# JohannesErnst/WeaSAL

Measured on AMD Instinct MI355X. Metric: points/sec fwd+bwd KPFCNN on DALES spheres; achieved HBM GB/s on KPConv gather, higher is better.
Workload: dtype f32; 1 GPU; DALES_PseudoLabel KP-FCNN, in_radius=10m, 50k pts/sphere, batch=8, fp32, step = GPU pyramid + fwd + loss + bwd + SGD; contrast_loss term included (trainer_PseudoLabel.py:204-208); pyramid of the next batch overlapped on a second stream; parallelism=dp1, dist_world_size=1, allreduce_bytes=0

## Files before the change

### include/weasal_hip.h

```cpp
#ifndef WEASAL_HIP_H
#define WEASAL_HIP_H

#include <stdint.h>

#ifdef __cplusplus
extern "C" {
#endif

typedef enum {
    WS_OK = 0,
    WS_ERR_INVALID = 1,
    WS_ERR_UNSUPPORTED = 2,
    WS_ERR_HIP = 3,
    WS_ERR_EMPTY = 4,
    WS_ERR_CAPACITY = 5
} ws_status;

enum { WS_INFLUENCE_LINEAR = 0, WS_INFLUENCE_CONSTANT = 1, WS_INFLUENCE_GAUSSIAN = 2 };
enum { WS_AGGREGATION_SUM = 0, WS_AGGREGATION_CLOSEST = 1 };

const char* ws_last_error(void);
int64_t ws_launch_count(void);
const char* ws_version(void);
int ws_device_count(void);
// ... 382 lines not shown
                      int32_t lut_n, const float* class_w, const float* grad_loss, const float* wsum, float* dlogits, int64_t ldd,
                      void* stream);
int ws_sgd_step(float* const* h_params, const float* const* h_grads, float* const* h_bufs, const int64_t* h_sizes, int32_t count,
                float lr, float momentum, float weight_decay, float clip_value, int32_t first, void* stream);

int ws_kpconv_deform_prepare(const float* offset_features, int64_t n, int32_t od, const float* kernel_points, int32_t k,
                             float extent, int32_t modulated, float* deformed_kp, float* modulations, float* kp4, float* kp_rmax,
                             void* stream);
int ws_kpconv_deform_prepare_bwd(const float* d_kp4, const float* d_deformed_kp, const float* kp4, int64_t n, int32_t od, int32_t k,
                                 float extent, int32_t modulated, float* d_offset_features, void* stream);
int ws_kpconv_gather_fwd_def(const float* q_pts, int64_t nq, const float* s_pts, int64_t ns, const int64_t* inds, int32_t h,
                             const void* x, int32_t ci, const float* kp4, int32_t k, float extent, const int32_t* order,
                             void* wf, float* min_d2, int32_t rows_bf16, int32_t rows_sorted, void* stream);
int ws_kpconv_gather_fwd_ex(const float* q_pts, int64_t nq, const float* s_pts, int64_t ns, const int64_t* inds, int32_t h,
                            const void* x, int32_t ci, const float* kernel_points, int32_t k, const float* deformed_kp,
                            const float* modulations, float extent, int32_t influence, int32_t aggregation, const int32_t* order,
                            void* wf, float* min_d2, int32_t rows_bf16, int32_t rows_sorted, void* stream);
int ws_kpconv_gather_bwd_x_def(const float* q_pts, int64_t nq, const float* s_pts, int64_t ns, int32_t h,
                               const int32_t* t_offsets, const int32_t* t_pairs, const void* dwf, int32_t ci, const float* kp4,
                               int32_t k, float extent, const int32_t* order, void* dx, int32_t rows_bf16, void* stream);
int ws_kpconv_gather_bwd_x_grid_wide(const float* s_pts, int64_t ns, const void* grid_blob, int32_t nb, int64_t cells,
                                     const uint64_t* key_last, float radius, const void* dwf, int32_t ci,
                                     const float* kernel_points, int32_t k, const float* kp4, const float* kp_rmax, float extent,
                                     const int32_t* order, const int64_t* rows, int32_t rows_h, void* dx, int32_t rows_bf16,
                                     void* stream);
int ws_kpconv_gather_bwd_geom_def(const float* q_pts, int64_t nq, const float* s_pts, int64_t ns, const int64_t* inds, int32_t h,
                                  const void* x, int32_t ci, const void* dwf, const float* kp4, int32_t k, const float* d_min_d2,
                                  float extent, const int32_t* order, float* d_kp4, int32_t rows_bf16, int32_t rows_sorted,
                                  void* stream);
int ws_kpconv_layer_fwd_fused(const float* q_pts, int64_t nq, const float* s_pts, int64_t ns, const int64_t* inds, int32_t h,
                              const float* x, int32_t ci, const float* kernel_points, int32_t k, float extent,
                              const int32_t* order, const float* weights, int32_t co, const float* bias, int32_t act, float slope,
                              float* out, void* stream);
int ws_kpconv_gather_fwd_variant(int32_t ci, int32_t mode, int32_t influence, int32_t aggregation, int32_t rows_bf16,
                                 int32_t rows_sorted, char* out, int32_t cap);
enum {
    WS_GATHER_FWD = 0, WS_GATHER_BWD_X = 1, WS_GATHER_BWD_GEOM = 2, WS_GATHER_BWD_X_GRID = 3,
    WS_GATHER_FWD_DEF = 4, WS_GATHER_BWD_X_DEF = 5, WS_GATHER_BWD_X_GRID_WIDE = 6, WS_GATHER_BWD_GEOM_DEF = 7
};
int ws_kpconv_gather_variant(int32_t op, int64_t nq, int64_t ns, int32_t ci, const void* rows_a, const void* rows_b, int32_t deformed,
                             int32_t modulated, int32_t influence, int32_t aggregation, int32_t rows_bf16, int32_t rows_sorted,
                             int32_t ordered, char* out, int32_t cap);
int ws_gemm_xb_variant(const float* x, int64_t m, int32_t k, int64_t ldx, const float* b, int64_t b_row_stride, int64_t b_col_stride,
                       int32_t n, const float* bias, const float* residual, int64_t ldr, const float* gate_y, int64_t ldg,
                       const uint8_t* mask, int64_t ldm, const float* y, int64_t ldy, const void* scratch, int64_t scratch_bytes,
                       char* out, int32_t cap);
int ws_gemm_xty_variant(const void* x, int64_t m, int32_t k, int64_t ldx, const void* y, int32_t n, int64_t ldy, float* out_m,
                        int64_t ldo, void* scratch, int32_t rows_bf16, char* out, int32_t cap);
int ws_act_bwd_colsum_variant(const float* dy, int64_t m, int32_t n, int64_t lddy, const float* y, int64_t ldy, const float* dz,
                              int64_t lddz, float* colsum, void* scratch, char* out, int32_t cap);
int ws_gemm_xbt_bf16_variant(int64_t m, int32_t k, int32_t n, const float* bias, const uint16_t* residual, int64_t ldr, const void* y,
                             int64_t ldy, int32_t out_f32, char* out, int32_t cap);
int ws_act_bwd_colsum_bf16_variant(int32_t dy_f32, int64_t m, int32_t n, float* colsum, void* scratch, char* out, int32_t cap);
int64_t ws_p2p_regularizer_scratch_bytes(int64_t n);
int ws_p2p_regularizer_fwd(const float* deformed_kp, const float* kp4, const float* min_d2, int64_t n, int32_t k, float extent,
                           float repulse_extent, float* out2, void* scratch, void* stream);
int ws_p2p_regularizer_bwd(const float* deformed_kp, const float* kp4, const float* min_d2, int64_t n, int32_t k, float extent,
                           float repulse_extent, const float* g2, float* d_min_d2, float* d_deformed_kp, void* stream);

#ifdef __cplusplus
}
#endif
#endif
```

### weasal_amd/_lib.py

```python
import ctypes as C
import os

_HERE = os.path.dirname(os.path.abspath(__file__))
LIB_PATH = os.path.join(_HERE, "libweasal_hip.so")

_vp = C.c_void_p
_i32 = C.c_int32
_i64 = C.c_int64
_f32 = C.c_float

SIGNATURES = {
    "ws_last_error": (C.c_char_p, []),
    "ws_version": (C.c_char_p, []),
    "ws_device_count": (C.c_int, []),
    "ws_kpconv_gather_fwd": (C.c_int, [_vp, _i64, _vp, _i64, _vp, _i32, _vp, _i32, _vp, _i32, _vp, _vp,
                                      _f32, _i32, _i32, _vp, _vp, _vp, _vp]),
    "ws_kpconv_gather_bwd_x": (C.c_int, [_vp, _i64, _vp, _i64, _vp, _i32, _vp, _vp, _vp, _i32, _vp, _i32,
                                        _vp, _vp, _f32, _i32, _i32, _vp, _vp, _vp]),
    "ws_kpconv_gather_bwd_geom": (C.c_int, [_vp, _i64, _vp, _i64, _vp, _i32, _vp, _i32, _vp, _vp, _i32,
                                           _vp, _vp, _vp, _f32, _i32, _i32, _vp, _vp, _vp]),
    "ws_transpose_scratch_bytes": (_i64, [_i64, _i32, _i64]),
    "ws_transpose_build": (C.c_int, [_vp, _i64, _i32, _i64, _vp, _vp, _vp, _vp]),
    "ws_max_pool_fwd": (C.c_int, [_vp, _i64, _i32, _vp, _i64, _i32, _vp, _vp, _vp]),
    "ws_max_pool_bwd": (C.c_int, [_vp, _vp, _i64, _i32, _i32, _vp, _vp, _i64, _vp, _vp]),
# ... 103 lines not shown
    "ws_anchor_scratch_bytes": (_i64, [_i64]),
    "ws_anchor_members_plan": (C.c_int, [_vp, _vp, _i64, _i32, _vp, _i64, C.c_double, _vp, _vp, _vp, _vp, _vp, _vp, _vp, _vp, _vp,
                                        _vp, _vp]),
    "ws_anchor_members_fill": (C.c_int, [_vp, _i64, _vp, _i64, C.c_double, _vp, _vp, _vp, _vp, _vp, _vp, _vp, _i64, _i64, _vp, _vp,
                                        _vp, _vp, _vp, _vp, _vp]),
    "ws_anchor_pairs_plan": (C.c_int, [_vp, _i64, _vp, _i64, C.c_double, _vp, _vp, _vp, _vp, _vp, _vp, _vp, _vp, _vp]),
    "ws_anchor_pairs_fill": (C.c_int, [_vp, _i64, _vp, _i64, C.c_double, _vp, _vp, _vp, _vp, _i64, _vp, _vp, _vp]),
    "ws_anchor_overlap_plan": (C.c_int, [_vp, _vp, _i64, _vp, _i64, _vp, _i64, _vp, _vp, _i64, _vp, _vp, _vp, _vp, _vp, _vp, _vp]),
    "ws_anchor_overlap_fill": (C.c_int, [_vp, _i64, _vp, _vp, _i64, _vp, _vp, _i64, _vp, _i64, _vp, _vp, _i64, _vp, _vp, _vp, _vp,
                                        _i64, _i64, _i64, _vp, _vp, _vp, _vp, _vp]),
    "ws_sampler_create": (C.c_int, [C.POINTER(_vp)]),
    "ws_sampler_destroy": (None, [_vp]),
    "ws_sampler_add_cloud": (C.c_int, [_vp, _vp, _vp, _i64, _vp, _vp, _i64, _vp]),
    "ws_sampler_state_bytes": (_i64, []),
    "ws_sampler_draw_bytes": (_i64, []),
    "ws_sampler_batch": (C.c_int, [_vp, _vp, _i32, _i32, _i64, C.c_double, _f32, C.c_uint64, C.c_uint64, _i32, _vp, _i32, _i32, _i32,
                                   _vp, _vp, _vp, _vp, _vp, _vp, _vp, _vp, _vp, _i64, _vp, _vp]),
    "ws_softmax_ce_scratch_bytes": (_i64, [_i64]),
    "ws_softmax_ce_fwd": (C.c_int, [_vp, _i64, _i32, _i64, _vp, _vp, _i32, _vp, _vp, _vp, _vp, _vp]),
    "ws_softmax_ce_bwd": (C.c_int, [_vp, _i64, _i32, _i64, _vp, _vp, _i32, _vp, _vp, _vp, _vp, _i64, _vp]),
    "ws_sgd_step": (C.c_int, [_vp, _vp, _vp, _vp, _i32, _f32, _f32, _f32, _f32, _i32, _vp]),
    "ws_kpconv_deform_prepare": (C.c_int, [_vp, _i64, _i32, _vp, _i32, _f32, _i32, _vp, _vp, _vp, _vp, _vp]),
    "ws_kpconv_gather_fwd_ex": (C.c_int, [_vp, _i64, _vp, _i64, _vp, _i32, _vp, _i32, _vp, _i32, _vp, _vp, _f32, _i32, _i32, _vp,
                                         _vp, _vp, _i32, _i32, _vp]),
    "ws_kpconv_deform_prepare_bwd": (C.c_int, [_vp, _vp, _vp, _i64, _i32, _i32, _f32, _i32, _vp, _vp]),
    "ws_kpconv_gather_fwd_def": (C.c_int, [_vp, _i64, _vp, _i64, _vp, _i32, _vp, _i32, _vp, _i32, _f32, _vp, _vp, _vp, _i32, _i32, _vp]),
    "ws_kpconv_gather_bwd_x_def": (C.c_int, [_vp, _i64, _vp, _i64, _i32, _vp, _vp, _vp, _i32, _vp, _i32, _f32, _vp, _vp, _i32, _vp]),
    "ws_kpconv_gather_bwd_x_grid_wide": (C.c_int, [_vp, _i64, _vp, _i32, _i64, _vp, _f32, _vp, _i32, _vp, _i32, _vp, _vp, _f32, _vp,
                                                   _vp, _i32, _vp, _i32, _vp]),
    "ws_kpconv_gather_bwd_geom_def": (C.c_int, [_vp, _i64, _vp, _i64, _vp, _i32, _vp, _i32, _vp, _vp, _i32, _vp, _f32, _vp, _vp,
                                                _i32, _i32, _vp]),
    "ws_kpconv_layer_fwd_fused": (C.c_int, [_vp, _i64, _vp, _i64, _vp, _i32, _vp, _i32, _vp, _i32, _f32, _vp, _vp, _i32, _vp, _i32, _f32,
                                           _vp, _vp]),
    "ws_kpconv_gather_fwd_variant": (C.c_int, [_i32, _i32, _i32, _i32, _i32, _i32, C.c_char_p, _i32]),
    "ws_kpconv_gather_variant": (C.c_int, [_i32, _i64, _i64, _i32, _vp, _vp, _i32, _i32, _i32, _i32, _i32, _i32, _i32, C.c_char_p, _i32]),
    "ws_gemm_xb_variant": (C.c_int, [_vp, _i64, _i32, _i64, _vp, _i64, _i64, _i32, _vp, _vp, _i64, _vp, _i64, _vp, _i64, _vp, _i64,
                                     _vp, _i64, C.c_char_p, _i32]),
    "ws_gemm_xty_variant": (C.c_int, [_vp, _i64, _i32, _i64, _vp, _i32, _i64, _vp, _i64, _vp, _i32, C.c_char_p, _i32]),
    "ws_act_bwd_colsum_variant": (C.c_int, [_vp, _i64, _i32, _i64, _vp, _i64, _vp, _i64, _vp, _vp, C.c_char_p, _i32]),
    "ws_gemm_xbt_bf16_variant": (C.c_int, [_i64, _i32, _i32, _vp, _vp, _i64, _vp, _i64, _i32, C.c_char_p, _i32]),
    "ws_act_bwd_colsum_bf16_variant": (C.c_int, [_i32, _i64, _i32, _vp, _vp, C.c_char_p, _i32]),
    "ws_p2p_regularizer_scratch_bytes": (_i64, [_i64]),
    "ws_p2p_regularizer_fwd": (C.c_int, [_vp, _vp, _vp, _i64, _i32, _f32, _f32, _vp, _vp, _vp]),
    "ws_p2p_regularizer_bwd": (C.c_int, [_vp, _vp, _vp, _i64, _i32, _f32, _f32, _vp, _vp, _vp, _vp]),
    "ws_timer_reset": (C.c_int, []),
    "ws_timer_count": (C.c_int, []),
    "ws_timer_read": (C.c_int, [_i32, _vp, _vp, _vp, _vp]),
    "ws_timer_read_layer": (C.c_int, [_i32, _vp]),
}

ENV_SWITCHES = (
    ("WEASAL_NB_WIDE_CAPS", "ws_nb_wide_caps"),
    ("WEASAL_CLOSEST_BWD_VEC", "ws_closest_bwd_vec"),
    ("WEASAL_GEMM_STAGED", "ws_gemm_staged"),
    ("WEASAL_GEMM_SHALLOW", "ws_gemm_shallow"),
)

_lib = None


class WeasalHipError(RuntimeError):
    pass


def lib():
    global _lib
# ... 43 lines not shown
```

### weasal_amd/csrc/blocks.hip

```cpp
#include <vector>

#include "ws_common.h"

extern "C" int ws_block_gates = 1;
extern "C" int ws_block_gather_residual = 1;
extern "C" int64_t ws_block_side_rows = 0;
extern "C" int ws_block_fused_infer = 1;
extern "C" int ws_block_pool_order = 1;

namespace {

struct Side {
    hipStream_t st = nullptr;
    hipEvent_t fork[3] = {nullptr, nullptr, nullptr};
    hipEvent_t join = nullptr;
};
int side_for_current_device(Side** out)
{
    static Side sides[16];
    int dev = 0;
    WS_HIP(hipGetDevice(&dev));
    WS_REQUIRE(dev >= 0 && dev < 16, "device index %d out of range", dev);
    Side& sd = sides[dev];
    if (!sd.st) {
        hipStream_t st;
        WS_HIP(hipStreamCreateWithFlags(&st, hipStreamNonBlocking));
        for (auto& e : sd.fork) WS_HIP(hipEventCreateWithFlags(&e, hipEventDisableTiming));
        WS_HIP(hipEventCreateWithFlags(&sd.join, hipEventDisableTiming));
        sd.st = st;
    }
    *out = &sd;
    return WS_OK;
}

struct Arena {
    char* base;
    int64_t cap, off;
    Arena(void* b, int64_t c) : base((char*)b), cap(c), off(0) {}
    template <typename T> T* take(int64_t count)
    {
// ... 80 lines not shown
    if (d->w1) t = max3(t, ws_gemm_xb_scratch_bytes(d->ns, d->in_dim, d->conv_in), 0);
    if (d->w2) t = max3(t, ws_gemm_xb_scratch_bytes(d->nq, d->conv_out, d->out_dim), d->ws ? ws_gemm_xb_scratch_bytes(d->nq, d->in_dim, d->out_dim) : 0);
    return t;
}

int kpblock_fwd(const ws_kpblock* d, Arena& ar, hipStream_t st, bool run)
{
    const int64_t nq = d->nq, ns = d->ns;
    const Lin l1{d->w1, d->conv_in, d->in_dim, d->in_dim}, l2{d->w2, d->out_dim, d->conv_out, d->conv_out},
        lsc{d->ws, d->out_dim, d->in_dim, d->in_dim};
    float* tr1 = d->w1 ? ar.take<float>(l1.tr_floats()) : nullptr;
    float* tr2 = d->w2 ? ar.take<float>(l2.tr_floats()) : nullptr;
    float* trs = d->ws ? ar.take<float>(lsc.tr_floats()) : nullptr;
    float* sc = (d->w2 && d->ws) ? ar.take<float>(nq * d->out_dim) : nullptr;
    const int64_t tmp_bytes = kpblock_tmp_fwd(d);
    void* tmp = ar.take<char>(tmp_bytes > 16 ? tmp_bytes : 16);
    if (!run) return WS_OK;
    if (nq == 0) return WS_OK;
    const float* x1 = d->feat;
    if (d->w1) {
        WS_TRY(linear_fwd(l1, d->feat, ns, d->in_dim, d->b1, nullptr, 0, 1, d->slope, d->x1, tr1, tmp, tmp_bytes, st));
        x1 = d->x1;
    }
    TimerRec rec{};
    if (d->timed) {
        WS_HIP(hipEventCreate(&rec.a));
        WS_HIP(hipEventCreate(&rec.b));
        rec.nq = nq; rec.h = d->h; rec.ci = d->conv_in;
        WS_HIP(hipEventRecord(rec.a, st));
    }
    float* x2 = d->w2 ? d->x2 : d->out;
    const bool one_launch = d->infer && d->conv_in == 32 && d->conv_out == 32 && !d->rows_sorted && ((uintptr_t)x1 & 15u) == 0 &&
                            ((uintptr_t)d->wk & 15u) == 0 && ((uintptr_t)x2 & 15u) == 0 && ws_block_fused_infer;
    if (one_launch) {
        WS_TRY(ws_kpconv_layer_fwd_fused(d->q_pts, nq, d->s_pts, ns, d->inds, d->h, x1, d->conv_in, d->kernel_points, d->k, d->extent,
                                         d->order_q, d->wk, d->conv_out, d->bk, 1, d->slope, x2, st));
        if (d->timed) WS_HIP(hipEventRecord(rec.b, st));
    } else {
        WS_REQUIRE(d->wf, "wf buffer missing");
        WS_TRY(ws_kpconv_gather_fwd_ex(d->q_pts, nq, d->s_pts, ns, d->inds, d->h, x1, d->conv_in, d->kernel_points, d->k, nullptr,
                                       nullptr, d->extent, WS_INFLUENCE_LINEAR, WS_AGGREGATION_SUM, d->order_q, d->wf, nullptr, 0,
                                       d->rows_sorted, st));
        if (d->timed) WS_HIP(hipEventRecord(rec.b, st));
        WS_TRY(ws_gemm_xb_epilogue_strided(d->wf, nq, d->k * d->conv_in, (int64_t)d->k * d->conv_in, d->wk, d->conv_out, 1, d->conv_out,
                                           d->bk, nullptr, 0, 1, d->slope, x2, d->conv_out, tmp, tmp_bytes, st));
    }
    if (d->timed) {
        WS_HIP(hipEventCreate(&rec.c));
        WS_HIP(hipEventRecord(rec.c, st));
        timer_recs().push_back(rec);
    }
    if (!d->w2) return WS_OK;
    const float* sc_in = d->feat;
    if (d->strided) {
        if (arg_bytes(d))
            WS_TRY(ws_priv_max_pool_fwd_u8(d->feat, ns, d->in_dim, d->inds, nq, d->h, d->pooled, reinterpret_cast<uint8_t*>(d->arg),
                                           ws_block_pool_order ? d->order_q : nullptr, st));
        else
            WS_TRY(ws_max_pool_fwd(d->feat, ns, d->in_dim, d->inds, nq, d->h, d->pooled, d->arg, st));
        sc_in = d->pooled;
    }
    const float* res = sc_in;
    int64_t ldr = d->in_dim;
    if (d->ws) {
        WS_TRY(linear_fwd(lsc, sc_in, nq, d->in_dim, d->bs, nullptr, 0, 0, 0.0f, sc, trs, tmp, tmp_bytes, st));
        res = sc;
        ldr = d->out_dim;
// ... 358 lines not shown
```

### weasal_amd/csrc/kpconv.hip

```cpp
#include "ws_common.h"
#include <algorithm>
#include "ws_grid.h"
#include "ws_bf16.h"

namespace {

constexpr float WS_SHADOW = 1e6f;

struct GeomParams {
    float extent;
    int influence;
    int aggregation;
    int deformable;
    const void* gate;
    float gate_slope;
    const int64_t* rows;
    int rows_h;
    const float4* kp4;
    const float* rmax;
    int cut;
    int ilv;
    int csplit;
};

// ... 396 lines not shown
                    flush(q, accumulate, maxlen);
                    accumulate = true;
                    h0 += 64;
                    continue;
                }
                total = 0; maxlen = 0;
            }
            auto minf = [&](int k, float d) {
                if (DEF && min_d2) {
                    float m = incol ? d : 3.4e38f;
#pragma unroll
                    for (int o = 32; o > 0; o >>= 1) m = fminf(m, __shfl_xor(m, o, 64));
                    if (lane == 0) min_d2[q * K + k] = h0 == 0 ? m : fminf(min_d2[q * K + k], m);
                }
            };
            kp_list<K, MODE>(nx, ny, nz, real, kp, g, inv_extent, row, 0u, nullptr, pool, segs, lane, total, maxlen, minf);
            if (total <= POOL) {
                flush(q, accumulate, maxlen);
                accumulate = true;
            } else {
                auto nomin = [&](int, float) {};
                for (int sub = 0; sub < 4; ++sub) {
                    total = 0; maxlen = 0;
                    kp_list<K, MODE>(nx, ny, nz, real && (lane >> 4) == sub, kp, g, inv_extent, row, 0u, nullptr, pool, segs,
                                     lane, total, maxlen, nomin);
                    flush(q, accumulate, maxlen);
                    accumulate = true;
                }
            }
        }
        q0 = q1; q1 = q2;
        idx0 = idx1; idx1 = idx2;
        p0x = p1x; p0y = p1y; p0z = p1z;
    }
}

typedef float f32x4v __attribute__((ext_vector_type(4)));
#ifndef WS_K3_GS
#define WS_K3_GS 4
#endif
#ifndef WS_FUSE_GS
#define WS_FUSE_GS 2
#endif

template <int NT, typename T> struct RowLoad;
template <int NT> struct RowLoad<NT, float> {
    static __device__ __forceinline__ void ld(const float* p, float (&v)[NT])
    {
        if constexpr (NT == 1) v[0] = *p;
        else if constexpr (NT == 2) { const float2 a = *reinterpret_cast<const float2*>(p); v[0] = a.x; v[1] = a.y; }
        else {
#pragma unroll
            for (int t = 0; t < NT; t += 4) {
                const float4 a = *reinterpret_cast<const float4*>(p + t);
                v[t] = a.x; v[t + 1] = a.y; v[t + 2] = a.z; v[t + 3] = a.w;
            }
        }
    }
    static __device__ __forceinline__ void st(float* p, const float (&v)[NT])
    {
        if constexpr (NT == 1) *p = v[0];
        else if constexpr (NT == 2) *reinterpret_cast<float2*>(p) = make_float2(v[0], v[1]);
        else {
#pragma unroll
            for (int t = 0; t < NT; t += 4) *reinterpret_cast<float4*>(p + t) = make_float4(v[t], v[t + 1], v[t + 2], v[t + 3]);
        }
// ... 1349 lines not shown
                    if (g.gate) {
                        a.x *= gq[c].x > 0.0f ? 1.0f : g.gate_slope; a.y *= gq[c].y > 0.0f ? 1.0f : g.gate_slope;
                        a.z *= gq[c].z > 0.0f ? 1.0f : g.gate_slope; a.w *= gq[c].w > 0.0f ? 1.0f : g.gate_slope;
                    }
                    if (VEC) {
                        if (chok[c]) st4(dst, a);
                    } else {
                        if (ch + 0 < ci) st1(dst + 0, a.x);
                        if (ch + 1 < ci) st1(dst + 1, a.y);
                        if (ch + 2 < ci) st1(dst + 2, a.z);
                        if (ch + 3 < ci) st1(dst + 3, a.w);
                    }
                }
            }
            wave_lds_order();
        }
    }
}

}

extern "C" int ws_kpconv_grid_sorted;
int ws_kpconv_grid_sorted = 0;

#include <cstdio>
#include <type_traits>

namespace {

constexpr int SPLIT_ROWS = 4096;
constexpr int SPLIT_NT = 4;
constexpr int GRID_INTERLEAVE = 512;

enum { GK_FWD_MFMA, GK_FWD_POOL, GK_BWD_X, GK_BWD_GEOM, GK_BWD_X_GRID, GK_BWD_X_GRIDW, GK_BWD_GEOM_DEF };
struct GatherPlan {
    int kernel;
    bool bf16;
    int n;
    int mode;
    bool def;
    bool vec;
    int pw;
    bool cut;
    int nch;
    bool sort;
    bool areg;
    int grid;
    int csplit, ilv, rows_sorted;
};

int nt_for_rows(int ci, const void* a, const void* b)
{
    const int nt = ci <= 16 ? 1 : (ci <= 32 ? 2 : (ci <= 64 ? 4 : (ci <= 128 ? 8 : 16)));
    return (ci % nt == 0 && (nt == 1 || (aligned16(a) && aligned16(b)))) ? nt : 1;
}
int group_ladder(int ci) { return ci <= 4 ? 1 : (ci <= 8 ? 2 : (ci <= 16 ? 4 : (ci <= 32 ? 8 : 16))); }
bool rows_vec4(bool bf16, int ci, const void* a, const void* b)
{
    return ci % 4 == 0 && (bf16 ? ws_row_aligned<bf16_t>(a) && ws_row_aligned<bf16_t>(b) : ws_row_aligned<float>(a) && ws_row_aligned<float>(b));
}
int rows_vec4_or_f32(bool bf16, int ci, const void* a, const void* b, bool& vec4)
{
    vec4 = rows_vec4(bf16, ci, a, b);
    WS_REQUIRE(!bf16 || vec4, "bf16 feature rows need ci %% 4 == 0 and 8-byte aligned rows (ci=%d)", ci);
    return WS_OK;
}
bool rigid_fast(bool deformed, bool modulated, int influence, int aggregation)
// ... 55 lines not shown

int bwd_geom_plan(bool bf16, int64_t nq, int32_t ci, const void* x, const void* dwf, GatherPlan& p)
{
    p = new_plan(GK_BWD_GEOM, bf16, nq);
    p.mode = 1; p.vec = rows_vec4(bf16, ci, x, dwf);
    return WS_OK;
}

int bwd_x_grid_plan(bool bf16, int64_t ns, int32_t ci, const void* dwf, const void* dx, int mode, bool ordered, GatherPlan& p)
{
    p = new_plan(GK_BWD_X_GRID, bf16, ns);
    p.n = group_ladder(ci); p.mode = mode; p.sort = ws_kpconv_grid_sorted != 0;
    grid_walk_plan(ns, ordered, p);
    return rows_vec4_or_f32(bf16, ci, dwf, dx, p.vec);
}

int bwd_x_gridw_plan(bool bf16, int64_t ns, int32_t ci, const void* dwf, const void* dx, bool deformed, bool ordered, GatherPlan& p)
{
    p = new_plan(GK_BWD_X_GRIDW, bf16, ns);
    p.n = group_ladder(ci); p.mode = deformed ? 2 : 0;
    p.nch = (p.n < 16 || ci <= 64) ? 1 : (ci <= 128 ? 2 : 4);
    grid_walk_plan(ns, ordered, p);
    return rows_vec4_or_f32(bf16, ci, dwf, dx, p.vec);
}

int bwd_geom_def_plan(bool bf16, int64_t nq, int32_t ci, const void* x, const void* dwf, bool rows_sorted, GatherPlan& p)
{
    p = new_plan(GK_BWD_GEOM_DEF, bf16, nq);
    if (ci % 16 != 0 || !aligned16(x) || !aligned16(dwf))
        return ws_fail(WS_ERR_UNSUPPORTED, "geometry backward on the matrix core needs ci %% 16 == 0 and 16-byte aligned rows (ci=%d)", ci);
    p.mode = 2; p.vec = true; p.cut = rows_sorted;
    p.areg = ci == 16 || ci == 32 || ci == 64 || ci == 128;
    p.n = p.areg ? ci / 4 : (ci % 128 == 0 ? 32 : (ci % 64 == 0 ? 16 : (ci % 32 == 0 ? 8 : 4)));
    return WS_OK;
}

void plan_text(const GatherPlan& p, char* out, size_t n)
{
    const char* t = p.bf16 ? "bf16" : "float";
    auto b = [](bool v) { return v ? "true" : "false"; };
    switch (p.kernel) {
    case GK_FWD_MFMA:
        snprintf(out, n, "kpconv_gather_fwd_mfma_kernel<NT=%d, MODE=%d, DEF=%s, VECROW=%s, T=%s, CUT=%s> grid=%d csplit=%d", p.n, p.mode,
                 b(p.def), b(p.vec), t, b(p.cut), p.grid, p.csplit);
        break;
    case GK_FWD_POOL:
        snprintf(out, n, "kpconv_gather_fwd_kernel<K=15, G=%d, MODE=%d, DEF=%s, VEC=%s, PW=%d, T=%s> grid=%d csplit=%d cut=%d", p.n, p.mode,
                 b(p.def), b(p.vec), p.pw, t, p.grid, p.csplit, p.rows_sorted);
        break;
    case GK_BWD_X:
        snprintf(out, n, "kpconv_gather_bwd_x_kernel<K=15, G=%d, MODE=%d, VEC=%s, T=%s> grid=%d", p.n, p.mode, b(p.vec), t, p.grid);
        break;
    case GK_BWD_GEOM:
        snprintf(out, n, "kpconv_gather_bwd_geom_kernel<K=15, T=%s> grid=%d vec4=%d", t, p.grid, p.vec ? 1 : 0);
        break;
    case GK_BWD_X_GRID:
        snprintf(out, n, "kpconv_gather_bwd_x_grid_kernel<K=15, G=%d, MODE=%d, VEC=%s, T=%s, SORT=%s> grid=%d ilv=%d", p.n, p.mode, b(p.vec),
                 t, b(p.sort), p.grid, p.ilv);
        break;
    case GK_BWD_X_GRIDW:
        snprintf(out, n, "kpconv_gather_bwd_x_gridw_kernel<K=15, G=%d, MODE=%d, VEC=%s, NCH=%d, T=%s> grid=%d ilv=%d", p.n, p.mode,
                 b(p.vec), p.nch, t, p.grid, p.ilv);
        break;
    default:
        snprintf(out, n, "kpconv_gather_bwd_geom_def_kernel<CK=%d, AREG=%s, T=%s, CUT=%s> grid=%d", p.n, b(p.areg), t, b(p.cut), p.grid);
    }
}

template <int... Vs> struct Pick { int v; };
using Flag = Pick<0, 1>;
template <typename F> void dispatch(F&& f) { f(); }
template <typename F, int... Vs, typename... Rest>
void dispatch(F&& f, Pick<Vs...> a, Rest... rest)
{
    (void)(((a.v == Vs) && (dispatch([&](auto... cs) { f(std::integral_constant<int, Vs>{}, cs...); }, rest...), true)) || ...);
}
template <int BF> using Row = std::conditional_t<BF != 0, bf16_t, float>;
int launched() { WS_LAUNCH_CHECK(); return WS_OK; }

struct GridView {
    const CloudGrid* grids;
    const int32_t* cell_start;
    const float4* sorted;
    const unsigned long long* key_last;
    float r2;
};
GridView grid_view(const void* grid_blob, int32_t nb, int64_t cells, const uint64_t* key_last, float radius)
{
    const char* base = (const char*)grid_blob;
    return GridView{(const CloudGrid*)base, (const int32_t*)(base + ws_grid_blob_cells_off(nb)),
                    (const float4*)(base + ws_grid_blob_sorted_off(nb, cells)), reinterpret_cast<const unsigned long long*>(key_last),
                    radius * radius};
}

void launch_fwd_mfma(const GatherPlan& p, void* stream, const float* q_pts, int64_t nq, const float* s_pts, int64_t ns, const int64_t* inds,
                     int32_t h, const void* x, int32_t ci, const float* kernel_points, const float* deformed_kp, const float* modulations,
// ... 202 lines not shown
    WS_REQUIRE(inds && x && dwf && kp4 && d_kp4 && aligned16(kp4) && aligned16(d_kp4), "NULL / unaligned argument");
    WS_REQUIRE(ns * (int64_t)ci < (1ll << 31) && nq * (int64_t)k * ci < (1ll << 31), "row offsets exceed 32 bits");
    GatherPlan p;
    if (int rc = bwd_geom_def_plan(rows_bf16 != 0, nq, ci, x, dwf, rows_sorted != 0, p)) return rc;
    dispatch([&](auto bf, auto ck, auto areg, auto cut) {
        using T = Row<bf.value>;
        kpconv_gather_bwd_geom_def_kernel<ck.value, areg.value != 0, T, cut.value != 0><<<p.grid, 256, 0, (hipStream_t)stream>>>(
            q_pts, nq, s_pts, ns, inds, h, (const T*)x, ci, (const T*)dwf, reinterpret_cast<const float4*>(kp4), d_min_d2, extent,
            reinterpret_cast<float4*>(d_kp4), order);
    }, Flag{p.bf16}, Pick<4, 8, 16, 32>{p.n}, Flag{p.areg}, Flag{p.cut});
    return launched();
}

int ws_kpconv_layer_fwd_fused(const float* q_pts, int64_t nq, const float* s_pts, int64_t ns, const int64_t* inds, int32_t h,
                              const float* x, int32_t ci, const float* kernel_points, int32_t k, float extent,
                              const int32_t* order, const float* weights, int32_t co, const float* bias, int32_t act, float slope,
                              float* out, void* stream)
{
    int rc = check_common(q_pts, nq, s_pts, ns, h, ci, k, extent, WS_INFLUENCE_LINEAR, WS_AGGREGATION_SUM);
    if (rc) return rc;
    if (ci != 32 || co != 32 || !aligned16(x) || !aligned16(weights) || !aligned16(out))
        return ws_fail(WS_ERR_UNSUPPORTED, "fused forward layer: 32 -> 32 channels, 16-byte aligned rows (got %d -> %d)", ci, co);
    if (nq == 0) return WS_OK;
    WS_REQUIRE(inds && x && kernel_points && weights && out, "NULL argument");
    WS_REQUIRE(ns * (int64_t)ci < (1ll << 31), "ns*ci exceeds the 32-bit row offsets of the gather");
    GeomParams g{extent, WS_INFLUENCE_LINEAR, WS_AGGREGATION_SUM, 0, nullptr, 0.0f, nullptr, 0, nullptr, nullptr, 0};
    FuseArgs fz{weights, bias, slope, act, out};
    kpconv_gather_fwd_mfma_kernel<2, 0, false, true, float, WS_FUSE_GS, false, true><<<ws_grid(nq, 4), 256, 0, (hipStream_t)stream>>>(
        q_pts, nq, s_pts, ns, inds, h, x, ci, kernel_points, nullptr, nullptr, g, nullptr, nullptr, order, fz);
    WS_LAUNCH_CHECK();
    return WS_OK;
}

int ws_kpconv_gather_variant(int32_t op, int64_t nq, int64_t ns, int32_t ci, const void* rows_a, const void* rows_b, int32_t deformed,
                             int32_t modulated, int32_t influence, int32_t aggregation, int32_t rows_bf16, int32_t rows_sorted,
                             int32_t ordered, char* out, int32_t cap)
{
    WS_REQUIRE(out && cap > 0 && ci >= 1 && nq >= 0 && ns >= 0, "bad argument");
    const bool bf = rows_bf16 != 0, def = deformed != 0, mod = modulated != 0, srt = rows_sorted != 0, ord = ordered != 0;
    const int mode = rigid_fast(def, mod, influence, aggregation) ? 0 : 1;
    GatherPlan p;
    int rc;
    switch (op) {
    case WS_GATHER_FWD: rc = fwd_plan(bf, nq, ci, rows_a, rows_b, def, mod, influence, aggregation, srt, p); break;
    case WS_GATHER_BWD_X: rc = bwd_x_plan(bf, ns, ci, rows_a, rows_b, mode, p); break;
    case WS_GATHER_BWD_GEOM: rc = bwd_geom_plan(bf, nq, ci, rows_a, rows_b, p); break;
    case WS_GATHER_BWD_X_GRID: rc = bwd_x_grid_plan(bf, ns, ci, rows_a, rows_b, mode, ord, p); break;
    case WS_GATHER_FWD_DEF: rc = fwd_def_plan(bf, nq, ci, rows_a, rows_b, srt, p); break;
    case WS_GATHER_BWD_X_DEF: rc = bwd_x_plan(bf, ns, ci, rows_a, rows_b, 2, p); break;
    case WS_GATHER_BWD_X_GRID_WIDE: rc = bwd_x_gridw_plan(bf, ns, ci, rows_a, rows_b, def, ord, p); break;
    case WS_GATHER_BWD_GEOM_DEF: rc = bwd_geom_def_plan(bf, nq, ci, rows_a, rows_b, srt, p); break;
    default: return ws_fail(WS_ERR_INVALID, "unknown gather operation %d", op);
    }
    if (rc == WS_OK) plan_text(p, out, (size_t)cap);
    return rc;
}

int ws_kpconv_gather_fwd_variant(int32_t ci, int32_t mode, int32_t influence, int32_t aggregation, int32_t rows_bf16,
                                 int32_t rows_sorted, char* out, int32_t cap)
{
    WS_REQUIRE(out && cap > 0 && ci >= 1, "bad argument");
    alignas(16) static const char row[16] = {};
    const bool bf = rows_bf16 != 0, srt = rows_sorted != 0;
    GatherPlan p;
    if (int rc = mode == 2 ? fwd_def_plan(bf, SPLIT_ROWS, ci, row, row, srt, p)
                           : fwd_plan(bf, SPLIT_ROWS, ci, row, row, mode != 0, false, influence, aggregation, srt, p))
        return rc;
    const char* t = bf ? "bf16" : "float";
    auto b = [](bool v) { return v ? "true" : "false"; };
    if (p.kernel == GK_FWD_MFMA)
        snprintf(out, (size_t)cap, "kpconv_gather_fwd_mfma_kernel<NT=%d, MODE=%d, DEF=%s, VECROW=true, %s, GS=default, CUT=%s>", p.n, p.mode,
                 b(p.def), t, b(p.cut));
    else
        snprintf(out, (size_t)cap, "kpconv_gather_fwd_kernel<K=15, G=%d, MODE=%d, DEF=%s, VEC=%s, PW=%d, %s>%s", p.n, p.mode, b(p.def),
                 b(p.vec), p.pw, t, (p.rows_sorted && p.mode == 0) ? " (sorted-row cutoff on)" : "");
    return WS_OK;
}

int ws_kpconv_gather_bwd_x(const float* q_pts, int64_t nq, const float* s_pts, int64_t ns,
                           const int64_t* inds, int32_t h, const int32_t* t_offsets, const int32_t* t_pairs,
                           const float* dwf, int32_t ci, const float* kernel_points, int32_t k,
                           const float* deformed_kp, const float* modulations, float extent,
                           int32_t influence, int32_t aggregation, const int32_t* order, float* dx, void* stream)
{
// ... 80 lines not shown
```

### weasal_amd/fused.py

```python
import ctypes as C
import os
import weakref

import torch

from . import _lib, ops
from ._lib import check, current_stream

FUSED_BLOCKS = os.environ.get("WEASAL_FUSED_BLOCKS", "1") != "0"
FUSED_INFER = os.environ.get("WEASAL_FUSED_INFER", "1") != "0"
_timed = False


_timed_min_rows = 0


def set_timed(on, min_rows=0):
    global _timed, _timed_min_rows
    _timed = bool(on)
    _timed_min_rows = int(min_rows)


_vp, _i32, _i64, _f32 = C.c_void_p, C.c_int32, C.c_int64, C.c_float


class KPBlockDesc(C.Structure):
    _fields_ = [("q_pts", _vp), ("nq", _i64), ("s_pts", _vp), ("ns", _i64), ("inds", _vp), ("h", _i32),
                ("kernel_points", _vp), ("k", _i32), ("extent", _f32), ("order_q", _vp), ("order_s", _vp),
                ("grid_blob", _vp), ("grid_nb", _i32), ("grid_cells", _i64), ("key_last", _vp), ("grid_radius", _f32),
                ("grid_overflow", _vp), ("t_offsets", _vp), ("t_pairs", _vp),
                ("in_dim", _i32), ("conv_in", _i32), ("conv_out", _i32), ("out_dim", _i32), ("strided", _i32),
                ("slope", _f32),
                ("w1", _vp), ("b1", _vp), ("wk", _vp), ("bk", _vp), ("w2", _vp), ("b2", _vp), ("ws", _vp), ("bs", _vp),
                ("feat", _vp), ("x1", _vp), ("wf", _vp), ("x2", _vp), ("pooled", _vp), ("arg", _vp), ("out", _vp),
                ("dout", _vp), ("dfeat", _vp), ("dw1", _vp), ("db1", _vp), ("dwk", _vp), ("dbk", _vp), ("dw2", _vp),
                ("db2", _vp), ("dws", _vp), ("timed", _i32), ("rows_sorted", _i32), ("infer", _i32), ("dout_pregated", _i32),
                ("gate_dfeat", _i32), ("dfeat_add", _vp)]


class UpUnaryDesc(C.Structure):
    _fields_ = [("xc", _vp), ("nc", _i64), ("c_up", _i32), ("skip", _vp), ("nf", _i64), ("c_skip", _i32),
                ("ups", _vp), ("h_up", _i32), ("t_offsets", _vp), ("t_pairs", _vp),
                ("w", _vp), ("ldw", _i64), ("b", _vp), ("out_dim", _i32), ("relu", _i32), ("slope", _f32),
                ("yc", _vp), ("out", _vp), ("dout", _vp), ("dxc", _vp), ("dskip", _vp), ("dw", _vp), ("db", _vp),
                ("drop_p", _f32), ("drop_seed", C.c_uint64), ("dout_pregated", _i32), ("gate_dxc", _i32)]


_GATES_SET = False


def _bind():
    global _GATES_SET
    lib = _lib.lib()
    if not _GATES_SET:
        C.c_int.in_dll(lib, "ws_block_gates").value = 0 if os.environ.get("WEASAL_BLOCK_GATES", "1") == "0" else 1
        C.c_int.in_dll(lib, "ws_block_fused_infer").value = 1 if FUSED_INFER else 0
        C.c_int.in_dll(lib, "ws_block_gather_residual").value = 0 if os.environ.get("WEASAL_BLOCK_GATHER_RESIDUAL", "1") == "0" else 1
        C.c_int.in_dll(lib, "ws_block_pool_order").value = 0 if os.environ.get("WEASAL_POOL_ORDER", "1") == "0" else 1
        if "WEASAL_BLOCK_SIDE_ROWS" in os.environ:
            C.c_int64.in_dll(lib, "ws_block_side_rows").value = int(os.environ["WEASAL_BLOCK_SIDE_ROWS"])
        _GATES_SET = True
    return lib


def timer_records(layer=False):
    lib = _bind()
    out = []
    nq, h, ci, ms, ml = _i64(), _i32(), _i32(), _f32(), _f32()
    for i in range(lib.ws_timer_count()):
        check(lib.ws_timer_read(i, C.byref(nq), C.byref(h), C.byref(ci), C.byref(ms)))
        if layer:
            check(lib.ws_timer_read_layer(i, C.byref(ml)))
            out.append((nq.value, h.value, ci.value, ms.value, ml.value))
        else:
            out.append((nq.value, h.value, ci.value, ms.value))
    return out


def timer_reset():
    _bind().ws_timer_reset()


def _p(t):
    return None if t is None else t.data_ptr()


def _scratch(nbytes, device):
    return torch.empty(max(int(nbytes), 256), dtype=torch.uint8, device=device)

# ... 360 lines not shown
```

Before: 31.75 million points/s.

## Fuse input-layer KPConv gather with weight GEMM, bias and activation in one kernel

Adds a dedicated kernel for the first KPConv layer (1-4 input channels) that computes the kernel-point weighted features per query in registers, stages them in LDS, and multiplies by the layer weights with bias and leaky ReLU inside the same launch. It also writes the weighted features to wf for backward. The block forward path takes this kernel by default when conv_in <= 4, replacing the separate gather and GEMM launches and the round trip of the intermediate through memory. In exchange, each query's tiny GEMM runs on scalar FMAs in LDS rather than a tuned GEMM, and the wf writes are scattered.

```diff
diff --git a/include/weasal_hip.h b/include/weasal_hip.h
--- a/include/weasal_hip.h
+++ b/include/weasal_hip.h
@@ -438,11 +438,20 @@
                               const float* x, int32_t ci, const float* kernel_points, int32_t k, float extent,
                               const int32_t* order, const float* weights, int32_t co, const float* bias, int32_t act, float slope,
                               float* out, void* stream);
+int ws_kpconv_input_layer_fwd(const float* q_pts, int64_t nq, const float* s_pts, int64_t ns, const int64_t* inds, int32_t h,
+                              const void* x, int32_t ci, const float* kernel_points, int32_t k, const float* deformed_kp,
+                              const float* modulations, float extent, int32_t influence, int32_t aggregation, const int32_t* order,
+                              int32_t rows_bf16, int32_t rows_sorted, const float* weights, int32_t co, const float* bias, int32_t act,
+                              float slope, float* wf, float* out, int32_t group_width, int32_t grid, void* stream);
+int ws_kpconv_input_layer_variant(int64_t nq, int32_t ci, int32_t co, int32_t deformed, int32_t modulated, int32_t influence,
+                                  int32_t aggregation, int32_t rows_bf16, int32_t rows_sorted, int32_t group_width, int32_t grid,
+                                  char* out, int32_t cap);
 int ws_kpconv_gather_fwd_variant(int32_t ci, int32_t mode, int32_t influence, int32_t aggregation, int32_t rows_bf16,
                                  int32_t rows_sorted, char* out, int32_t cap);
 enum {
     WS_GATHER_FWD = 0, WS_GATHER_BWD_X = 1, WS_GATHER_BWD_GEOM = 2, WS_GATHER_BWD_X_GRID = 3,
-    WS_GATHER_FWD_DEF = 4, WS_GATHER_BWD_X_DEF = 5, WS_GATHER_BWD_X_GRID_WIDE = 6, WS_GATHER_BWD_GEOM_DEF = 7
+    WS_GATHER_FWD_DEF = 4, WS_GATHER_BWD_X_DEF = 5, WS_GATHER_BWD_X_GRID_WIDE = 6, WS_GATHER_BWD_GEOM_DEF = 7,
+    WS_GATHER_INPUT_LAYER = 8
 };
 int ws_kpconv_gather_variant(int32_t op, int64_t nq, int64_t ns, int32_t ci, const void* rows_a, const void* rows_b, int32_t deformed,
                              int32_t modulated, int32_t influence, int32_t aggregation, int32_t rows_bf16, int32_t rows_sorted,
diff --git a/weasal_amd/_lib.py b/weasal_amd/_lib.py
--- a/weasal_amd/_lib.py
+++ b/weasal_amd/_lib.py
@@ -159,6 +159,9 @@
                                                 _i32, _i32, _vp]),
     "ws_kpconv_layer_fwd_fused": (C.c_int, [_vp, _i64, _vp, _i64, _vp, _i32, _vp, _i32, _vp, _i32, _f32, _vp, _vp, _i32, _vp, _i32, _f32,
                                            _vp, _vp]),
+    "ws_kpconv_input_layer_fwd": (C.c_int, [_vp, _i64, _vp, _i64, _vp, _i32, _vp, _i32, _vp, _i32, _vp, _vp, _f32, _i32, _i32, _vp, _i32, _i32,
+                                           _vp, _i32, _vp, _i32, _f32, _vp, _vp, _i32, _i32, _vp]),
+    "ws_kpconv_input_layer_variant": (C.c_int, [_i64, _i32, _i32, _i32, _i32, _i32, _i32, _i32, _i32, _i32, _i32, C.c_char_p, _i32]),
     "ws_kpconv_gather_fwd_variant": (C.c_int, [_i32, _i32, _i32, _i32, _i32, _i32, C.c_char_p, _i32]),
     "ws_kpconv_gather_variant": (C.c_int, [_i32, _i64, _i64, _i32, _vp, _vp, _i32, _i32, _i32, _i32, _i32, _i32, _i32, C.c_char_p, _i32]),
     "ws_gemm_xb_variant": (C.c_int, [_vp, _i64, _i32, _i64, _vp, _i64, _i64, _i32, _vp, _vp, _i64, _vp, _i64, _vp, _i64, _vp, _i64,
diff --git a/weasal_amd/csrc/blocks.hip b/weasal_amd/csrc/blocks.hip
--- a/weasal_amd/csrc/blocks.hip
+++ b/weasal_amd/csrc/blocks.hip
@@ -6,6 +6,7 @@
 extern "C" int ws_block_gather_residual = 1;
 extern "C" int64_t ws_block_side_rows = 0;
 extern "C" int ws_block_fused_infer = 1;
+extern "C" int ws_block_input_fused = 1;
 extern "C" int ws_block_pool_order = 1;
 
 namespace {
@@ -152,7 +153,17 @@
     float* x2 = d->w2 ? d->x2 : d->out;
     const bool one_launch = d->infer && d->conv_in == 32 && d->conv_out == 32 && !d->rows_sorted && ((uintptr_t)x1 & 15u) == 0 &&
                             ((uintptr_t)d->wk & 15u) == 0 && ((uintptr_t)x2 & 15u) == 0 && ws_block_fused_infer;
-    if (one_launch) {
+    int input_rc = WS_ERR_UNSUPPORTED;
+    if (!one_launch && ws_block_input_fused && d->conv_in <= 4) {
+        WS_REQUIRE(d->wf || d->infer, "wf buffer missing");
+        input_rc = ws_kpconv_input_layer_fwd(d->q_pts, nq, d->s_pts, ns, d->inds, d->h, x1, d->conv_in, d->kernel_points, d->k, nullptr,
+                                             nullptr, d->extent, WS_INFLUENCE_LINEAR, WS_AGGREGATION_SUM, d->order_q, 0, d->rows_sorted,
+                                             d->wk, d->conv_out, d->bk, 1, d->slope, d->infer ? nullptr : d->wf, x2, 0, 0, st);
+        if (input_rc != WS_OK && input_rc != WS_ERR_UNSUPPORTED) return input_rc;
+    }
+    if (input_rc == WS_OK) {
+        if (d->timed) WS_HIP(hipEventRecord(rec.b, st));
+    } else if (one_launch) {
         WS_TRY(ws_kpconv_layer_fwd_fused(d->q_pts, nq, d->s_pts, ns, d->inds, d->h, x1, d->conv_in, d->kernel_points, d->k, d->extent,
                                          d->order_q, d->wk, d->conv_out, d->bk, 1, d->slope, x2, st));
         if (d->timed) WS_HIP(hipEventRecord(rec.b, st));
diff --git a/weasal_amd/csrc/kpconv.hip b/weasal_amd/csrc/kpconv.hip
--- a/weasal_amd/csrc/kpconv.hip
+++ b/weasal_amd/csrc/kpconv.hip
@@ -452,6 +452,174 @@
         q0 = q1; q1 = q2;
         idx0 = idx1; idx1 = idx2;
         p0x = p1x; p0y = p1y; p0z = p1z;
+    }
+}
+
+template <int GW, int CI>
+__global__ __launch_bounds__(256) void kpconv_input_layer_fwd_kernel(
+    const float* __restrict__ q_pts, int64_t nq, const float* __restrict__ s_pts, int64_t ns,
+    const int64_t* __restrict__ inds, int h, const float* __restrict__ x, const float* __restrict__ kernel_points,
+    float extent, int cut, const int32_t* __restrict__ order, const float* __restrict__ weights, int co,
+    const float* __restrict__ bias, int act, float slope, float* __restrict__ wf, float* __restrict__ out)
+{
+    constexpr int K = 15, KC = K * CI;
+    constexpr int QW = 64 / GW;
+    constexpr int KPL = (K + GW - 1) / GW;
+    constexpr int KCP = (KC + 3) & ~3;
+    constexpr int ROW = KCP + 4;
+    static_assert(QW % 4 == 0 && QW <= 32 && CI >= 1 && CI <= 4, "group width 2, 4, 8 or 16; 1..4 channels");
+    __shared__ __attribute__((aligned(16))) float wl[KCP * 64];
+    __shared__ __attribute__((aligned(16))) float slab_all[4][QW * ROW];
+    const int wave = __builtin_amdgcn_readfirstlane(threadIdx.x >> 6);
+    const int lane = threadIdx.x & 63;
+    const int j = lane % GW, grp = lane / GW;
+    float* slab = slab_all[wave];
+
+    for (int e = threadIdx.x; e < KCP * 64; e += 256) {
+        const int kc = e >> 6, c = e & 63;
+        wl[e] = (kc < KC && c < co) ? weights[kc * co + c] : 0.0f;
+    }
+    __syncthreads();
+
+    float kx[KPL], ky[KPL], kz[KPL];
+#pragma unroll
+    for (int t = 0; t < KPL; ++t) {
+        const int k = j + GW * t;
+        kx[t] = ky[t] = kz[t] = 1e18f;
+        if (k < K) { kx[t] = kernel_points[3 * k]; ky[t] = kernel_points[3 * k + 1]; kz[t] = kernel_points[3 * k + 2]; }
+    }
+    float cut2 = 3.4e38f;
+    if (cut) {
+        float rr = 0.0f;
+        for (int k = 0; k < K; ++k) {
+            const float a = kernel_points[3 * k], b = kernel_points[3 * k + 1], c = kernel_points[3 * k + 2];
+            rr = fmaxf(rr, (a * a + b * b) + c * c);
+        }
+        const float R = (__builtin_sqrtf(rr) + extent) * 1.0001f;
+        cut2 = R * R;
+    }
+    const float inv_extent = 1.0f / extent;
+    const float bl = (bias && lane < co) ? bias[lane] : 0.0f;
+
+    struct Nb { float px, py, pz, f[CI]; };
+    const int64_t n_items = (nq + QW - 1) / QW;
+    int64_t ibeg, iend;
+    ws_block_range(n_items, ibeg, iend);
+    for (int64_t item = ibeg + wave; item < iend; item += 4) {
+        const int64_t pos = item * QW + grp;
+        int64_t q = -1;
+        if (pos < nq) {
+            q = order ? (int64_t)order[pos] : pos;
+            if (q < 0 || q >= nq) q = -1;
+        }
+        const bool qok = q >= 0;
+        const int64_t ql = qok ? q : 0;
+        const float qx = q_pts[3 * ql], qy = q_pts[3 * ql + 1], qz = q_pts[3 * ql + 2];
+        const int64_t* __restrict__ row = inds + ql * (int64_t)h;
+        const int hm = h - 1;
+        bool done = !qok;
+        auto raw = [&](int col) -> int64_t { return row[min(col, hm)]; };
+        auto valid = [&](int64_t v, int col) -> int { return (v >= 0 && v < ns && col < h && !done) ? (int)v : -1; };
+        auto load_nb = [&](int idx, Nb& n) {
+            const int64_t r = max(idx, 0);
+            const float* p = s_pts + 3 * r;
+            const float* f = x + CI * r;
+            n.px = p[0]; n.py = p[1]; n.pz = p[2];
+#pragma unroll
+            for (int c = 0; c < CI; ++c) n.f[c] = f[c];
+        };
+        float acc[KPL][CI];
+#pragma unroll
+        for (int t = 0; t < KPL; ++t)
+#pragma unroll
+            for (int c = 0; c < CI; ++c) acc[t][c] = 0.f;
+        auto step = [&](const Nb& n, int idx) {
+            const bool live = idx >= 0;
+            const float nx = n.px - qx, ny = n.py - qy, nz = n.pz - qz;
+            if (cut && live && (nx * nx + ny * ny) + nz * nz > cut2) done = true;
+            float f[CI];
+#pragma unroll
+            for (int c = 0; c < CI; ++c) f[c] = live ? n.f[c] : 0.0f;
+#pragma unroll
+            for (int t = 0; t < KPL; ++t) {
+                const float dx = nx - kx[t], dy = ny - ky[t], dz = nz - kz[t];
+                const float d = (dx * dx + dy * dy) + dz * dz;
+                const float w = fmaxf(1.0f - __builtin_amdgcn_sqrtf(d) * inv_extent, 0.0f);
+#pragma unroll
+                for (int c = 0; c < CI; ++c) acc[t][c] = fmaf(w, f[c], acc[t][c]);
+            }
+        };
+
+        Nb A, B;
+        int64_t rA = raw(0), rB = raw(1);
+        int iA = valid(rA, 0);
+        load_nb(iA, A);
+        rA = raw(2);
+        for (int col = 0; col < h; col += 2) {
+            const int iB = valid(rB, col + 1);
+            load_nb(iB, B);
+            rB = raw(col + 3);
+            step(A, iA);
+            iA = valid(rA, col + 2);
+            load_nb(iA, A);
+            rA = raw(col + 4);
+            step(B, iB);
+            if (cut && __ballot(!done) == 0ull) break;
+        }
+
+        wave_lds_order();
+#pragma unroll
+        for (int t = 0; t < KPL; ++t) {
+            const int k = j + GW * t;
+            if (k < K) {
+#pragma unroll
+                for (int c = 0; c < CI; ++c) slab[grp * ROW + k * CI + c] = acc[t][c];
+            }
+        }
+        if (j == 0) {
+#pragma unroll
+            for (int e = KC; e < KCP; ++e) slab[grp * ROW + e] = 0.0f;
+            slab[grp * ROW + KCP] = __int_as_float((int)q);
+        }
+        wave_lds_order();
+
+        if (wf) {
+            for (int e = lane; e < QW * KC; e += 64) {
+                const int g = e / KC, kc = e - g * KC;
+                const int qi = __float_as_int(slab[g * ROW + KCP]);
+                if (qi >= 0) wf[(int64_t)qi * KC + kc] = slab[g * ROW + kc];
+            }
+        }
+        for (int g0 = 0; g0 < QW; g0 += 4) {
+            int qi[4];
+            float a[4];
+#pragma unroll
+            for (int u = 0; u < 4; ++u) { qi[u] = __float_as_int(slab[(g0 + u) * ROW + KCP]); a[u] = 0.f; }
+            if ((qi[0] & qi[1] & qi[2] & qi[3]) < 0) continue;
+#pragma unroll 2
+            for (int kc4 = 0; kc4 < KCP; kc4 += 4) {
+                float4 v[4];
+#pragma unroll
+                for (int u = 0; u < 4; ++u) v[u] = *reinterpret_cast<const float4*>(&slab[(g0 + u) * ROW + kc4]);
+#pragma unroll
+                for (int t = 0; t < 4; ++t) {
+                    const float wv = wl[(kc4 + t) * 64 + lane];
+#pragma unroll
+                    for (int u = 0; u < 4; ++u) {
+                        const float s = t == 0 ? v[u].x : (t == 1 ? v[u].y : (t == 2 ? v[u].z : v[u].w));
+                        a[u] = fmaf(s, wv, a[u]);
+                    }
+                }
+            }
+#pragma unroll
+            for (int u = 0; u < 4; ++u) {
+                if (qi[u] >= 0 && lane < co) {
+                    float o = a[u] + bl;
+                    if (act) o = o > 0.0f ? o : o * slope;
+                    out[(int64_t)qi[u] * co + lane] = o;
+                }
+            }
+        }
     }
 }
 
@@ -1867,7 +2035,7 @@
 constexpr int SPLIT_NT = 4;
 constexpr int GRID_INTERLEAVE = 512;
 
-enum { GK_FWD_MFMA, GK_FWD_POOL, GK_BWD_X, GK_BWD_GEOM, GK_BWD_X_GRID, GK_BWD_X_GRIDW, GK_BWD_GEOM_DEF };
+enum { GK_FWD_MFMA, GK_FWD_POOL, GK_BWD_X, GK_BWD_GEOM, GK_BWD_X_GRID, GK_BWD_X_GRIDW, GK_BWD_GEOM_DEF, GK_FWD_INPUT };
 struct GatherPlan {
     int kernel;
     bool bf16;
@@ -1989,6 +2157,21 @@
     p.mode = 2; p.vec = true; p.cut = rows_sorted;
     p.areg = ci == 16 || ci == 32 || ci == 64 || ci == 128;
     p.n = p.areg ? ci / 4 : (ci % 128 == 0 ? 32 : (ci % 64 == 0 ? 16 : (ci % 32 == 0 ? 8 : 4)));
+    return WS_OK;
+}
+
+constexpr int INPUT_GW = 4;
+int input_plan(bool bf16, int64_t nq, int32_t ci, int32_t co, bool deformed, bool modulated, int32_t influence, int32_t aggregation,
+               bool rows_sorted, int32_t gw, int32_t grid, GatherPlan& p)
+{
+    if (bf16 || !rigid_fast(deformed, modulated, influence, aggregation) || ci > 4 || co < 1 || co > 64)
+        return ws_fail(WS_ERR_UNSUPPORTED, "input layer in one launch: f32 rows, rigid kernel, linear influence, sum, ci <= 4, co <= 64 "
+                                           "(got ci=%d co=%d bf16=%d)", ci, co, bf16 ? 1 : 0);
+    if (gw == 0) gw = INPUT_GW;
+    WS_REQUIRE((gw == 2 || gw == 4 || gw == 8 || gw == 16) && grid >= 0, "group width 2 / 4 / 8 / 16 (got %d)", gw);
+    p = new_plan(GK_FWD_INPUT, false, ws_ceil_div(ws_ceil_div(nq, 64 / gw), 2));
+    p.n = gw; p.nch = ci; p.rows_sorted = rows_sorted;
+    if (grid > 0) p.grid = grid;
     return WS_OK;
 }
 
@@ -2019,6 +2202,9 @@
         snprintf(out, n, "kpconv_gather_bwd_x_gridw_kernel<K=15, G=%d, MODE=%d, VEC=%s, NCH=%d, T=%s> grid=%d ilv=%d", p.n, p.mode,
                  b(p.vec), p.nch, t, p.grid, p.ilv);
         break;
+    case GK_FWD_INPUT:
+        snprintf(out, n, "kpconv_input_layer_fwd_kernel<GW=%d, CI=%d> grid=%d cut=%d", p.n, p.nch, p.grid, p.rows_sorted);
+        break;
     default:
         snprintf(out, n, "kpconv_gather_bwd_geom_def_kernel<CK=%d, AREG=%s, T=%s, CUT=%s> grid=%d", p.n, b(p.areg), t, b(p.cut), p.grid);
     }
@@ -2287,6 +2473,42 @@
     return WS_OK;
 }
 
+int ws_kpconv_input_layer_fwd(const float* q_pts, int64_t nq, const float* s_pts, int64_t ns, const int64_t* inds, int32_t h,
+                              const void* x, int32_t ci, const float* kernel_points, int32_t k, const float* deformed_kp,
+                              const float* modulations, float extent, int32_t influence, int32_t aggregation, const int32_t* order,
+                              int32_t rows_bf16, int32_t rows_sorted, const float* weights, int32_t co, const float* bias, int32_t act,
+                              float slope, float* wf, float* out, int32_t group_width, int32_t grid, void* stream)
+{
+    if (int rc = check_common(q_pts, nq, s_pts, ns, h, ci, k, extent, influence, aggregation)) return rc;
+    GatherPlan p;
+    if (int rc = input_plan(rows_bf16 != 0, nq, ci, co, deformed_kp != nullptr, modulations != nullptr, influence, aggregation,
+                            rows_sorted != 0, group_width, grid, p))
+        return rc;
+    if (nq == 0) return WS_OK;
+    if (ns == 0) return ws_fail(WS_ERR_UNSUPPORTED, "input layer in one launch: no support points");
+    WS_REQUIRE(inds && x && kernel_points && weights && out, "NULL argument");
+    WS_REQUIRE(ns * (int64_t)ci < (1ll << 31) && nq * (int64_t)k * ci < (1ll << 31) && nq * (int64_t)co < (1ll << 40),
+               "row offsets exceed their range");
+    dispatch([&](auto gw, auto cc) {
+        kpconv_input_layer_fwd_kernel<gw.value, cc.value><<<p.grid, 256, 0, (hipStream_t)stream>>>(
+            q_pts, nq, s_pts, ns, inds, h, (const float*)x, kernel_points, extent, p.rows_sorted, order, weights, co, bias, act, slope, wf, out);
+    }, Pick<2, 4, 8, 16>{p.n}, Pick<1, 2, 3, 4>{p.nch});
+    return launched();
+}
+
+int ws_kpconv_input_layer_variant(int64_t nq, int32_t ci, int32_t co, int32_t deformed, int32_t modulated, int32_t influence,
+                                  int32_t aggregation, int32_t rows_bf16, int32_t rows_sorted, int32_t group_width, int32_t grid,
+                                  char* out, int32_t cap)
+{
+    WS_REQUIRE(out && cap > 0 && ci >= 1 && nq >= 0, "bad argument");
+    GatherPlan p;
+    if (int rc = input_plan(rows_bf16 != 0, nq, ci, co, deformed != 0, modulated != 0, influence, aggregation, rows_sorted != 0,
+                            group_width, grid, p))
+        return rc;
+    plan_text(p, out, (size_t)cap);
+    return WS_OK;
+}
+
 int ws_kpconv_gather_variant(int32_t op, int64_t nq, int64_t ns, int32_t ci, const void* rows_a, const void* rows_b, int32_t deformed,
                              int32_t modulated, int32_t influence, int32_t aggregation, int32_t rows_bf16, int32_t rows_sorted,
                              int32_t ordered, char* out, int32_t cap)
@@ -2305,6 +2527,7 @@
     case WS_GATHER_BWD_X_DEF: rc = bwd_x_plan(bf, ns, ci, rows_a, rows_b, 2, p); break;
     case WS_GATHER_BWD_X_GRID_WIDE: rc = bwd_x_gridw_plan(bf, ns, ci, rows_a, rows_b, def, ord, p); break;
     case WS_GATHER_BWD_GEOM_DEF: rc = bwd_geom_def_plan(bf, nq, ci, rows_a, rows_b, srt, p); break;
+    case WS_GATHER_INPUT_LAYER: rc = input_plan(bf, nq, ci, 64, def, mod, influence, aggregation, srt, 0, 0, p); break;
     default: return ws_fail(WS_ERR_INVALID, "unknown gather operation %d", op);
     }
     if (rc == WS_OK) plan_text(p, out, (size_t)cap);
diff --git a/weasal_amd/fused.py b/weasal_amd/fused.py
--- a/weasal_amd/fused.py
+++ b/weasal_amd/fused.py
@@ -9,6 +9,7 @@
 
 FUSED_BLOCKS = os.environ.get("WEASAL_FUSED_BLOCKS", "1") != "0"
 FUSED_INFER = os.environ.get("WEASAL_FUSED_INFER", "1") != "0"
+INPUT_LAYER_FUSED = os.environ.get("WEASAL_INPUT_LAYER_FUSED", "1") != "0"
 _timed = False
 
 
@@ -55,6 +56,7 @@
     if not _GATES_SET:
         C.c_int.in_dll(lib, "ws_block_gates").value = 0 if os.environ.get("WEASAL_BLOCK_GATES", "1") == "0" else 1
         C.c_int.in_dll(lib, "ws_block_fused_infer").value = 1 if FUSED_INFER else 0
+        C.c_int.in_dll(lib, "ws_block_input_fused").value = 1 if INPUT_LAYER_FUSED else 0
         C.c_int.in_dll(lib, "ws_block_gather_residual").value = 0 if os.environ.get("WEASAL_BLOCK_GATHER_RESIDUAL", "1") == "0" else 1
         C.c_int.in_dll(lib, "ws_block_pool_order").value = 0 if os.environ.get("WEASAL_POOL_ORDER", "1") == "0" else 1
         if "WEASAL_BLOCK_SIDE_ROWS" in os.environ:
```

Result: slower. 31.42 million points/s (-1.0%).
